# ai-forever/Kandinsky-2

Measured on NVIDIA B200. Metric: unet_denoising_steps_per_sec, higher is better.
Workload: dtype f16

## Files before the change

### kandinsky-2_b200/csrc/k2_api.cu

```cuda
#include <stdio.h>
#include <stdlib.h>
#include <string.h>

#include <algorithm>
#include <atomic>
#include <mutex>

#include "../../include/k2b200.h"
#include "k2_internal.h"

namespace k2 {

static thread_local std::string g_err;
static std::atomic<long long> g_launches{0};
static int g_force_bn = 0;
static int g_force_split = 0;
static int g_force_2cta = 0;
static int g_tail_split = 0;
static int g_attn_stagger = 1200;
static int g_attn_poly = 0;
static int g_pdl = 0;
static int g_halo_mode = 0;


// ... 99 lines not shown
        if (better) {
          best_tiles[k] = tiles;
          bn[k] = tn;
          bw[k] = tw;
          bh[k] = th;
        }
      }
    }
  }
  const int k = (!single_image_only && best_tiles[1] * 100 <= best_tiles[0] * 85) ? 1 : 0;
  TN = bn[k];
  TW = bw[k];
  TH = bh[k];
}


struct ConvPlan {
  int TN, TH, TW, tiles_w, tiles_h, tiles_n, m_tiles;
  int halo_pitch, halo_bo;
  int m_tiles_phase;
  int BN, two_cta, splits;
  int fuse_stats, row_groups;
  int es;
  int tail_first, tail_count, tail_split, tail_kps;
};

constexpr long long TAIL_FLAG_BYTES = 64 << 10;

static void plan_conv(int NB, int H, int W, bool any9, int kchunks, int Cout, int out_mode, bool has_workspace,
                      long long workspace_bytes, bool want_gn, ConvPlan& pl, const int* cfg = nullptr, bool up2 = false,
                      bool w_batched = false) {
  const int g_force_bn = (cfg && cfg[0]) ? cfg[0] : k2::g_force_bn;
  const int g_force_2cta = (cfg && cfg[1]) ? cfg[1] : k2::g_force_2cta;
  const int g_force_split = (cfg && cfg[2]) ? cfg[2] : k2::g_force_split;
  pl.es = (cfg && cfg[3]) ? cfg[3] : k2::g_conv_epi_sets;
  pl.halo_pitch = 0;
  pl.halo_bo = 0;
  if (g_halo_mode > 0 && any9 && W % 8 == 0 && H % 16 == 0 && out_mode == 0 && Cout > 64 && g_force_2cta != 1) {
    pl.halo_pitch = (g_halo_mode <= 2) ? 10 : 16;
    pl.halo_bo = (g_halo_mode == 2 || g_halo_mode == 4) ? 1 : 0;
  }
  if (pl.halo_pitch) {
    pl.TN = 1;
    pl.TH = 16;
    pl.TW = 8;
  } else {
// ... 42 lines not shown
    long long best = -1;
    int best_bn = BN ? BN : 256, best_sp = 1;
    for (int ci = 0; ci < 3; ++ci) {
      const int bn = BN ? BN : cand[ci];
      if (BN && ci > 0) break;
      for (int sp = 1; sp <= 8; ++sp) {
        if (g_force_split > 0 && sp != g_force_split) continue;
        if (pl.halo_pitch && sp > 1) continue;
        if (!split_ok(sp)) continue;
        const long long c = model(bn, sp, two_cta != 0);
        if (best < 0 || c < best) {
          best = c;
          best_bn = bn;
          best_sp = sp;
        }
      }
    }
    BN = best_bn;
    splits = best_sp;
  }
  pl.BN = BN;
  pl.two_cta = two_cta;
  pl.splits = splits;
  if (up2) {
    pl.m_tiles_phase = two_cta ? (pl.m_tiles + 1) / 2 * 2 : pl.m_tiles;
  }

  pl.tail_first = pl.tail_count = pl.tail_kps = 0;
  pl.tail_split = 1;
  if (g_tail_split && two_cta && splits == 1 && !pl.halo_pitch && out_mode == 0 && Cout % 64 == 0 && BN % 64 == 0 && has_workspace) {
    const int m_pairs = ((up2 ? 4 * pl.m_tiles_phase : pl.m_tiles) + 1) / 2;
    const int units = m_pairs * ((Cout + BN - 1) / BN);
    const int P = num_sms() / 2;
    const int R = units % P;
    if (R > 0 && kchunks >= 16) {
      long long L = (static_cast<long long>(R) * kchunks + P - 1) / P;
      L = std::max<long long>(L, (kchunks + 2) / 3);
      int max_parts = 1;
      for (int t = 0; t < R; ++t) {
        const long long first = static_cast<long long>(t) * kchunks / L;
        const long long last = std::min((static_cast<long long>(t + 1) * kchunks - 1) / L, (static_cast<long long>(R) * kchunks - 1) / L);
        max_parts = std::max(max_parts, static_cast<int>(last - first + 1));
      }
      const long long buf_bytes = static_cast<long long>(R) * 2 * 3 * 128 * BN * 4;
      const long long flag_bytes = static_cast<long long>(R) * 2 * 3 * 8 * 4;
      const long long saved_cycles = (kchunks - L) * (2LL * BN + 60);
      if ((saved_cycles >= 26000 || (g_tail_split == 2 && L < kchunks)) && max_parts <= 4 && buf_bytes <= workspace_bytes / 2 - TAIL_FLAG_BYTES &&
          flag_bytes <= TAIL_FLAG_BYTES) {
        pl.tail_first = units - R;
        pl.tail_count = R;
        pl.tail_split = 4;
        pl.tail_kps = static_cast<int>(L);
      }
    }
  }

  pl.fuse_stats = 0;
  pl.row_groups = 0;
  if (want_gn && out_mode == 0 && Cout % 8 == 0) {
    if (splits == 1 && BN >= 64 && Cout % 64 == 0 && (pl.TN == 1 || pl.TH * pl.TW == 16)) {
      pl.fuse_stats = 1;
      pl.row_groups = ((pl.TN == 1) ? pl.m_tiles : NB * pl.tiles_h * pl.tiles_w) * (up2 ? 4 : 1);
    } else if (splits > 1 && (static_cast<long long>(H) * W) % 16 == 0) {
      pl.fuse_stats = 2;
      pl.row_groups = static_cast<int>(M_total / 16);
    }
  }
}

static thread_local int g_last_tail_split = 1;
static void plan_to_info(const ConvPlan& pl, int* info) {
  g_last_tail_split = pl.tail_split;
  if (!info) return;
  info[0] = pl.BN; info[1] = pl.two_cta; info[2] = pl.splits; info[3] = pl.m_tiles; info[4] = pl.TN;
  info[5] = pl.fuse_stats; info[6] = pl.row_groups;
}

}

using namespace k2;

extern "C" {

const char* k2_last_error(void) { return g_err.c_str(); }
int k2_version(void) { return 100; }
long long k2_launch_count(void) { return g_launches.load(); }
int k2_conv_last_tail_split(void) { return g_last_tail_split; }
void k2_reset_launch_count(void) { g_launches.store(0); }
int k2_set_tuning(int key, int value) {
  if (key == 0) {
    g_force_bn = value;
    return 0;
  }
  if (key == 1) {
    g_force_split = value;
    return 0;
  }
// ... 42 lines not shown
    return 0;
  }

  return fail("k2_set_tuning: unknown key");
}

int k2_conv_gemm(const K2ConvSrc* srcs, int nsrc, int NB, int H, int W, const void* w_packed, int w_rows,
                 int Ktot, int ldw, int Cout, const float* bias, const void* residual, int ldr, void* out, int ldo,
                 int out_mode, void* workspace, long long workspace_bytes, float* gn_partial, int* info,
                 k2_stream_t stream) {
  return k2_conv_gemm_cfg(srcs, nsrc, NB, H, W, w_packed, w_rows, Ktot, ldw, Cout, bias, residual, ldr, out, ldo, out_mode,
                          workspace, workspace_bytes, gn_partial, info, nullptr, 0, stream);
}

int k2_conv_gemm_cfg(const K2ConvSrc* srcs, int nsrc, int NB, int H, int W, const void* w_packed, int w_rows,
                     int Ktot, int ldw, int Cout, const float* bias, const void* residual, int ldr, void* out, int ldo,
                     int out_mode, void* workspace, long long workspace_bytes, float* gn_partial, int* info,
                     const int* cfg, long long w_batch_stride, k2_stream_t stream) {
  K2_REQUIRE(w_batch_stride >= 0 && w_batch_stride % 8 == 0, "conv_gemm_cfg: w_batch_stride must be a multiple of 8 elements");
  const bool w_batched = w_batch_stride > 0;
  if (cfg) {
    K2_REQUIRE(cfg[0] == 0 || cfg[0] == 16 || cfg[0] == 64 || cfg[0] == 128 || cfg[0] == 192 || cfg[0] == 256,
               "conv_gemm_cfg: N tile must be 0, 16, 64, 128, 192 or 256");
    K2_REQUIRE(cfg[1] >= 0 && cfg[1] <= 2 && cfg[2] >= 0 && cfg[2] <= 8 && cfg[3] >= 0 && cfg[3] <= 2,
               "conv_gemm_cfg: pair mode in 0..2, splits in 0..8, epilogue sets in 0..2");
  }
  K2_REQUIRE(nsrc >= 1 && nsrc <= 3, "conv_gemm: 1..3 sources");
  K2_REQUIRE(NB > 0 && H > 0 && W > 0 && Cout > 0, "conv_gemm: bad geometry");
  K2_REQUIRE(w_rows >= Cout, "conv_gemm: w_rows < Cout");
  K2_REQUIRE(Ktot % 64 == 0, "conv_gemm: Ktot must be a multiple of 64");
  if (ldw == 0) ldw = Ktot;
  K2_REQUIRE(ldw >= Ktot && ldw % 8 == 0 && (reinterpret_cast<uintptr_t>(w_packed) & 15) == 0,
             "conv_gemm: weight row stride / alignment");
  ConvGemmParams p;
  memset(&p, 0, sizeof p);
  p.NB = NB;
  p.H = H;
  p.W = W;
  bool any9 = false;
  int kchunks = 0;
  const bool up2 = srcs[0].taps == 4;
  if (up2) {
    K2_REQUIRE(nsrc == 1 && out_mode == 0 && residual == nullptr && H % 2 == 0 && W % 2 == 0,
               "conv_gemm: a taps == 4 source (3x3 conv over its nearest-2x upsampling) must be the only source, with fp16 "
               "output, no residual and even output H, W");
    H /= 2;
    W /= 2;
    p.H = H;
// ... 61 lines not shown
  }
  p.n_tiles = (Cout + BN - 1) / BN;
  p.Cout = Cout;
  {
    uint64_t dims[3] = {static_cast<uint64_t>(Ktot), static_cast<uint64_t>(w_rows), static_cast<uint64_t>(w_batched ? NB : 1)};
    uint64_t str[2] = {static_cast<uint64_t>(ldw) * 2,
                       (w_batched ? static_cast<uint64_t>(w_batch_stride) : static_cast<uint64_t>(ldw) * w_rows) * 2};
    uint32_t box[3] = {64, static_cast<uint32_t>(two_cta ? BN / 2 : BN), 1};
    if (encode_tmap_f16(&p.tmB, w_packed, 3, dims, str, box)) return -1;
  }
  p.bias = bias;
  p.residual = reinterpret_cast<const __half*>(residual);
  p.ldr = ldr;
  p.out = out;
  p.ldo = ldo;
  p.out_mode = (splits > 1) ? 2 : out_mode;
  p.gn_part = (fuse_stats == 1) ? reinterpret_cast<float2*>(gn_partial) : nullptr;
  p.gn_mode = (fuse_stats == 1) ? (p.TN == 1 ? 1 : 2) : 0;
  if (out_mode == 0) {
    K2_REQUIRE(ldo % 8 == 0 && (reinterpret_cast<uintptr_t>(out) & 15) == 0, "conv_gemm: out alignment");
    if (residual)
      K2_REQUIRE(ldr % 8 == 0 && (reinterpret_cast<uintptr_t>(residual) & 15) == 0, "conv_gemm: residual alignment");
  }
  int rc = launch_conv_gemm(p, BN, pl.es, static_cast<cudaStream_t>(stream));
  if (rc == 0) g_launches.fetch_add(1, std::memory_order_relaxed);
  if (rc == 0 && splits > 1) {
    rc = launch_splitk_finalize(p.ws, splits, p.M_total, Cout, bias, p.residual, ldr, reinterpret_cast<__half*>(out), ldo,
                                fuse_stats == 2 ? reinterpret_cast<float2*>(gn_partial) : nullptr,
                                static_cast<cudaStream_t>(stream));
    if (rc == 0) g_launches.fetch_add(1, std::memory_order_relaxed);
  }
  return rc;
}

int k2_conv_plan(int NB, int H, int W, int taps, int Ktot, int Cout, int out_mode, long long workspace_bytes,
                 int want_gn_partial, int* info) {
  K2_REQUIRE(NB > 0 && H > 0 && W > 0 && Cout > 0 && info, "conv_plan: bad arguments");
  K2_REQUIRE(Ktot > 0 && Ktot % 64 == 0, "conv_plan: Ktot must be a positive multiple of 64");
  ConvPlan pl;
  plan_conv(NB, H, W, taps == 9, Ktot / 64, Cout, out_mode, workspace_bytes > 0, workspace_bytes, want_gn_partial != 0, pl);
  plan_to_info(pl, info);
  return 0;
}

}
```

### kandinsky-2_b200/csrc/k2_common.cuh

```cuda
#pragma once
#include <cuda.h>
#include <cuda_fp16.h>
#include <cuda_runtime.h>
#include <stdint.h>
#include <stdio.h>

namespace k2 {

__device__ __forceinline__ uint32_t smem_u32(const void* p) {
  return static_cast<uint32_t>(__cvta_generic_to_shared(p));
}

__device__ __forceinline__ uint32_t lane_id() { return threadIdx.x & 31; }

__device__ __forceinline__ bool elect_one() {
  uint32_t pred = 0;
  asm volatile(
      "{\n"
      ".reg .b32 rx;\n"
      ".reg .pred px;\n"
      "elect.sync rx|px, 0xffffffff;\n"
      "selp.b32 %0, 1, 0, px;\n"
      "}\n"
      : "=r"(pred));
// ... 237 lines not shown
      "cp.async.bulk.tensor.2d.cta_group::2.shared::cluster.global.mbarrier::complete_tx::bytes [%0], [%1, {%3, "
      "%4}], [%2];"
      ::"r"(smem_u32(dst)),
      "l"(reinterpret_cast<uint64_t>(tm)), "r"(smem_u32(bar) & kPeerBitMask), "r"(c0), "r"(c1)
      : "memory");
}
__device__ __forceinline__ void tma2_load_3d(void* dst, const CUtensorMap* tm, uint64_t* bar, int c0, int c1, int c2) {
  asm volatile(
      "cp.async.bulk.tensor.3d.cta_group::2.shared::cluster.global.mbarrier::complete_tx::bytes [%0], [%1, {%3, "
      "%4, %5}], [%2];"
      ::"r"(smem_u32(dst)),
      "l"(reinterpret_cast<uint64_t>(tm)), "r"(smem_u32(bar) & kPeerBitMask), "r"(c0), "r"(c1), "r"(c2)
      : "memory");
}
__device__ __forceinline__ void tma2_load_4d(void* dst, const CUtensorMap* tm, uint64_t* bar, int c0, int c1,
                                             int c2, int c3) {
  asm volatile(
      "cp.async.bulk.tensor.4d.cta_group::2.shared::cluster.global.mbarrier::complete_tx::bytes [%0], [%1, {%3, "
      "%4, %5, %6}], [%2];"
      ::"r"(smem_u32(dst)),
      "l"(reinterpret_cast<uint64_t>(tm)), "r"(smem_u32(bar) & kPeerBitMask), "r"(c0), "r"(c1), "r"(c2), "r"(c3)
      : "memory");
}
__device__ __forceinline__ void tmem_alloc2(uint32_t* smem_dst, uint32_t ncols) {
  asm volatile("tcgen05.alloc.cta_group::2.sync.aligned.shared::cta.b32 [%0], %1;" ::"r"(smem_u32(smem_dst)),
               "r"(ncols)
               : "memory");
}
__device__ __forceinline__ void tmem_relinquish2() {
  asm volatile("tcgen05.relinquish_alloc_permit.cta_group::2.sync.aligned;" ::: "memory");
}
__device__ __forceinline__ void tmem_dealloc2(uint32_t taddr, uint32_t ncols) {
  asm volatile("tcgen05.dealloc.cta_group::2.sync.aligned.b32 %0, %1;" ::"r"(taddr), "r"(ncols) : "memory");
}
__device__ __forceinline__ void umma2_f16(uint32_t tmem_d, uint64_t adesc, uint64_t bdesc, uint32_t idesc,
                                          uint32_t accumulate) {
  asm volatile(
      "{\n"
      ".reg .pred p;\n"
      "setp.ne.b32 p, %4, 0;\n"
      "tcgen05.mma.cta_group::2.kind::f16 [%0], %1, %2, %3, p;\n"
      "}\n" ::"r"(tmem_d),
      "l"(adesc), "l"(bdesc), "r"(idesc), "r"(accumulate)
      : "memory");
}
__device__ __forceinline__ void umma2_commit_mc(uint64_t* bar, uint16_t mask) {
// ... 117 lines not shown
```

### kandinsky-2_b200/csrc/k2_conv_gemm.cu

```cuda
#include <stdio.h>

#include "k2_common.cuh"
#include "k2_internal.h"

namespace k2 {

namespace {

constexpr int BM = 128;
constexpr int BK = 64;
constexpr int A_STAGE_BYTES = BM * BK * 2;

constexpr int EPI_STAGE_FLOATS = 32 * 33;
constexpr int EPI_BYTES = 4 * EPI_STAGE_FLOATS * 4 + 4 * 256 * 4;

template <int BN>
struct Cfg {
  static constexpr int B_STAGE_BYTES = BN * BK * 2;
  static constexpr int STAGE_BYTES = A_STAGE_BYTES + B_STAGE_BYTES;
  static constexpr int STAGES = (BN >= 256) ? 4 : (BN >= 192 ? 5 : (BN >= 128 ? 6 : 8));
  static constexpr int TMEM_COLS = (2 * BN <= 32) ? 32 : (2 * BN <= 64 ? 64 : (2 * BN <= 128 ? 128 : (2 * BN <= 256 ? 256 : 512)));
  static constexpr int BAR_BYTES = 256;
  static constexpr int STAT_BYTES = EPI_BYTES;
  static constexpr int SMEM_BYTES = STAGES * STAGE_BYTES + BAR_BYTES + STAT_BYTES + 1024;
// ... 511 lines not shown
      acc ^= 1;
      if (acc == 0) acc_phase ^= 1;
    }
  }

  tc_fence_before();
  __syncthreads();
  if (warp_idx == 2) {
    tc_fence_after();
    tmem_dealloc(tmem_base, C::TMEM_COLS);
  }
}

template <int BN, int ES = 1>
struct Cfg2 {
  static constexpr int B_STAGE_BYTES = (BN / 2) * BK * 2;
  static constexpr int STAGE_BYTES = A_STAGE_BYTES + B_STAGE_BYTES;
  static constexpr int STAGES = ((BN >= 256) ? 6 : (BN >= 192 ? 7 : 8)) - (ES - 1);
  static constexpr int TMEM_COLS = 512;
  static constexpr int SMEM_BYTES = STAGES * STAGE_BYTES + 256 + ES * EPI_BYTES + 1024;
  static constexpr int THREADS = 128 + 128 * ES;
};

template <int BN, int ES = 1, bool TAIL = false>
__global__ void __cluster_dims__(2, 1, 1) __launch_bounds__(128 + 128 * ES, 1)
conv_gemm2_kernel(const __grid_constant__ ConvGemmParams p) {
  using C = Cfg2<BN, ES>;
  extern __shared__ uint8_t smem_raw[];
  uint8_t* smem = reinterpret_cast<uint8_t*>((reinterpret_cast<uintptr_t>(smem_raw) + 1023) &
                                             ~static_cast<uintptr_t>(1023));
  uint64_t* full_bar = reinterpret_cast<uint64_t*>(smem + C::STAGES * C::STAGE_BYTES);
  uint64_t* empty_bar = full_bar + C::STAGES;
  uint64_t* tmem_full = empty_bar + C::STAGES;
  uint64_t* tmem_empty = tmem_full + 2;
  uint32_t* tmem_ptr = reinterpret_cast<uint32_t*>(tmem_empty + 2);
  float* stat_smem = reinterpret_cast<float*>(smem + C::STAGES * C::STAGE_BYTES + 256);

  const int warp_idx = threadIdx.x >> 5;
  const int lane = threadIdx.x & 31;
  const uint32_t rank = cluster_ctarank();
  const int pair = blockIdx.x >> 1;
  const int num_pairs = gridDim.x >> 1;

  if (warp_idx == 0 && lane == 0) {
    tma_prefetch_desc(&p.tmB);
    for (int s = 0; s < 3; ++s)
      if (p.seg_taps[s]) tma_prefetch_desc(&p.tmA[s]);
  }
  if (warp_idx == 1 && lane == 0) {
    for (int i = 0; i < C::STAGES; ++i) {
      mbar_init(&full_bar[i], 1);
      mbar_init(&empty_bar[i], 1);
    }
    for (int i = 0; i < 2; ++i) {
      mbar_init(&tmem_full[i], 1);
      mbar_init(&tmem_empty[i], 8 * ES);
    }
    fence_barrier_init();
  }
  if (warp_idx == 2) {
    tmem_alloc2(tmem_ptr, C::TMEM_COLS);
    tmem_relinquish2();
  }
  tc_fence_before();
  cluster_sync_all();
  tc_fence_after();
  const uint32_t tmem_base = *tmem_ptr;
  pdl_wait();
  pdl_launch();

  const int m_pairs = (p.m_tiles + 1) >> 1;
  const int total_tiles = TAIL ? p.tail_first + 2 * num_pairs : m_pairs * p.n_tiles * p.splits;
  auto decode_item = [&](int item, int& tile, int& part, int& nparts, int& split, int& k0, int& k1) -> bool {
    if (TAIL && item >= p.tail_first) {
      const int idx = item - p.tail_first;
      const int sub = idx / num_pairs, i = idx - sub * num_pairs;
      const int nk = p.num_k_chunks, L = p.tail_kps;
      const int g0 = i * L, g1 = min(g0 + L, p.tail_count * nk);
      if (g0 >= g1) return false;
      int ta = g0 / nk;
      const int ka0 = g0 - ta * nk, ka1 = min(nk, ka0 + (g1 - g0));
      if (sub == 0) {
        k0 = ka0;
        k1 = ka1;
      } else {
        const int rest = (g1 - g0) - (ka1 - ka0);
        if (rest <= 0) return false;
        ++ta;
        k0 = 0;
        k1 = rest;
      }
      const int first_span = (ta * nk) / L;
      const int last_span = min(((ta + 1) * nk - 1) / L, (p.tail_count * nk - 1) / L);
      part = i - first_span;
      nparts = last_span - first_span + 1;
      tile = p.tail_first + ta;
      split = 0;
      return true;
    }
    tile = item;
    part = -1;
    nparts = 1;
    split = tile / (m_pairs * p.n_tiles);
    k0 = split * p.k_per_split;
    k1 = min(p.num_k_chunks, k0 + p.k_per_split);
    return true;
  };

  if (warp_idx == 0) {
    if (elect_one()) {
      int stage = 0;
      uint32_t ring_phase = 0;
      const uint32_t tx_bytes = 2u * (p.a_box_bytes + C::B_STAGE_BYTES);
      for (int item = pair; item < total_tiles; item += num_pairs) {
        int tile, part, nparts, split, k0, k1;
        if (!decode_item(item, tile, part, nparts, split, k0, k1)) continue;
        const int m_idx = (tile % m_pairs) * 2 + static_cast<int>(rank);
        const int n_idx = (tile / m_pairs) % p.n_tiles;
        int n0, y0, x0, phase;
        decode_m_tile(p, m_idx, n0, y0, x0, phase);
        const int kb = phase * p.num_k_chunks;
        int s = 0, rem = k0;
        while (rem >= p.seg_taps[s] * p.seg_kchunks[s]) {
          rem -= p.seg_taps[s] * p.seg_kchunks[s];
          ++s;
        }
        int tap = rem / p.seg_kchunks[s];
        int c = rem - tap * p.seg_kchunks[s];
        for (int kc = k0; kc < k1; ++kc) {
          const int taps = p.seg_taps[s];
          const int dy = (taps == 9) ? (tap / 3 - 1) : (taps == 4 ? (tap >> 1) + (phase >> 1) - 1 : 0);
          const int dx = (taps == 9) ? (tap % 3 - 1) : (taps == 4 ? (tap & 1) + (phase & 1) - 1 : 0);
          mbar_wait(&empty_bar[stage], ring_phase ^ 1);
          uint8_t* sA = smem + stage * C::STAGE_BYTES;
          uint8_t* sB = sA + A_STAGE_BYTES;
          if (rank == 0) mbar_arrive_expect_tx(&full_bar[stage], tx_bytes);
          tma2_load_4d(sA, &p.tmA[s], &full_bar[stage], c * BK, x0 + dx, y0 + dy, n0);
          tma2_load_3d(sB, &p.tmB, &full_bar[stage], (kb + kc) * BK, n_idx * BN + static_cast<int>(rank) * (BN / 2),
                       p.w_batched ? n0 : 0);
          if (++stage == C::STAGES) {
            stage = 0;
            ring_phase ^= 1;
          }
          if (++c == p.seg_kchunks[s]) {
            c = 0;
            if (++tap == taps) {
              tap = 0;
              ++s;
            }
          }
        }
      }
    }
  } else if (warp_idx == 1) {
    if (rank == 0 && elect_one()) {
      constexpr uint32_t idesc = make_idesc_f16(256, BN, 0, 0);
      int stage = 0;
      uint32_t phase = 0;
      int acc = 0;
      uint32_t acc_phase = 0;
      for (int item = pair; item < total_tiles; item += num_pairs) {
        int tile, part, nparts, split, k0, k1;
        if (!decode_item(item, tile, part, nparts, split, k0, k1)) continue;
        mbar_wait(&tmem_empty[acc], acc_phase ^ 1);
        tc_fence_after();
        const uint32_t d_tmem = tmem_base + static_cast<uint32_t>(acc * 256);
        const int nk = k1 - k0;
        for (int kc = 0; kc < nk; ++kc) {
          mbar_wait(&full_bar[stage], phase);
          tc_fence_after();
          const uint32_t a_addr = smem_u32(smem + stage * C::STAGE_BYTES);
          const uint64_t adesc = make_sw128_desc(a_addr);
          const uint64_t bdesc = make_sw128_desc(a_addr + A_STAGE_BYTES);
#pragma unroll
          for (int k = 0; k < BK / 16; ++k)
            umma2_f16(d_tmem, adesc + static_cast<uint64_t>(k * 2), bdesc + static_cast<uint64_t>(k * 2), idesc,
                      (kc | k) != 0 ? 1u : 0u);
          umma2_commit_mc(&empty_bar[stage], 0x3);
          if (++stage == C::STAGES) {
            stage = 0;
            phase ^= 1;
          }
        }
        umma2_commit_mc(&tmem_full[acc], 0x3);
        acc ^= 1;
        if (acc == 0) acc_phase ^= 1;
      }
    }
  } else if (warp_idx >= 4) {
    const int ew = (ES == 1) ? warp_idx - 4 : (warp_idx & 3);
    const int es = (ES == 1) ? 0 : ((warp_idx - 4) >> 2);
    int acc = 0;
    uint32_t acc_phase = 0;
    const uint32_t leader_empty0 = mapa_u32(smem_u32(&tmem_empty[0]), 0);
    const uint32_t leader_empty1 = mapa_u32(smem_u32(&tmem_empty[1]), 0);
    for (int item = pair; item < total_tiles; item += num_pairs) {
      int tile, part, nparts, split, k0, k1;
      if (!decode_item(item, tile, part, nparts, split, k0, k1)) continue;
      const int m_idx = (tile % m_pairs) * 2 + static_cast<int>(rank);
      const int n_idx = (tile / m_pairs) % p.n_tiles;
      int n0, y0, x0, phase;
      decode_m_tile(p, m_idx, n0, y0, x0, phase);
      const int tail_role = (part < 0 || nparts == 1) ? 0 : (part > 0 ? 1 : 2);
      const int tail_slot = (part < 0) ? 0 : ((tile - p.tail_first) * 2 + static_cast<int>(rank)) * (p.tail_split - 1) + max(part - 1, 0);
      mbar_wait(&tmem_full[acc], acc_phase);
      tc_fence_after();
      epilogue_tile<BN, ES, TAIL>(p, tmem_base, acc * 256, ew, lane, n0, y0, x0, n_idx, split, m_idx, stat_smem, es, phase,
                                  tail_role, tail_slot, nparts - 1);
      tc_fence_before();
      __syncwarp();
      if (lane == 0) mbar_arrive_cluster(acc ? leader_empty1 : leader_empty0);
      acc ^= 1;
      if (acc == 0) acc_phase ^= 1;
    }
  }

  tc_fence_before();
  cluster_sync_all();
  if (warp_idx == 2) {
    tc_fence_after();
    tmem_dealloc2(tmem_base, C::TMEM_COLS);
  }
}

template <int BN, int ES, bool TAIL>
int launch_pair(const ConvGemmParams& p, cudaStream_t stream) {
  using C = Cfg2<BN, ES>;
  static bool attr_set = false;
  if (!attr_set) {
    K2_CHECK_CUDA(cudaFuncSetAttribute(conv_gemm2_kernel<BN, ES, TAIL>, cudaFuncAttributeMaxDynamicSharedMemorySize, C::SMEM_BYTES));
    attr_set = true;
  }
  const int m_pairs = (p.m_tiles + 1) / 2;
  const int total = m_pairs * p.n_tiles * p.splits;
  const int max_pairs = num_sms() / 2;
  const int pairs = (TAIL || total >= max_pairs) ? max_pairs : total;
  K2_CHECK_CUDA(launch_k(conv_gemm2_kernel<BN, ES, TAIL>, dim3(2 * pairs), dim3(C::THREADS), C::SMEM_BYTES, stream, p));
  return 0;
}
template <int BN>
int launch_bn2(const ConvGemmParams& p, cudaStream_t stream) {
  return p.tail_split > 1 ? launch_pair<BN, 1, true>(p, stream) : launch_pair<BN, 1, false>(p, stream);
}
template <int BN>
int launch_bn2e(const ConvGemmParams& p, cudaStream_t stream) {
  return p.tail_split > 1 ? launch_pair<BN, 2, true>(p, stream) : launch_pair<BN, 2, false>(p, stream);
}

template <int BN>
struct Cfg3 {
  static constexpr int A_STAGE = 36864;
  static constexpr int A_STAGES = 3;
  static constexpr int B_STAGE = (BN / 2) * BK * 2;
  static constexpr int B_STAGES = (BN >= 256) ? 4 : 5;
  static constexpr int BAR_OFF = A_STAGES * A_STAGE + B_STAGES * B_STAGE;
  static constexpr int STAT_OFF = BAR_OFF + 256;
  static constexpr int SMEM_BYTES = STAT_OFF + EPI_BYTES + 1024;
};

template <int BN>
__global__ void __cluster_dims__(2, 1, 1) __launch_bounds__(256, 1)
conv_gemm3_kernel(const __grid_constant__ ConvGemmParams p) {
  using C = Cfg3<BN>;
  extern __shared__ uint8_t smem_raw[];
  uint8_t* smem = reinterpret_cast<uint8_t*>((reinterpret_cast<uintptr_t>(smem_raw) + 1023) &
                                             ~static_cast<uintptr_t>(1023));
  uint8_t* smemB = smem + C::A_STAGES * C::A_STAGE;
  uint64_t* a_full = reinterpret_cast<uint64_t*>(smem + C::BAR_OFF);
  uint64_t* a_empty = a_full + C::A_STAGES;
// ... 265 lines not shown
  using C = Cfg<BN>;
  static bool attr_set = false;
  if (!attr_set) {
    K2_CHECK_CUDA(cudaFuncSetAttribute(conv_gemm_kernel<BN>, cudaFuncAttributeMaxDynamicSharedMemorySize,
                                       C::SMEM_BYTES));
    attr_set = true;
  }
  int total = p.m_tiles * p.n_tiles * p.splits;
  int grid = total < num_sms() ? total : num_sms();
  K2_CHECK_CUDA(launch_k(conv_gemm_kernel<BN>, dim3(grid), dim3(256), C::SMEM_BYTES, stream, p));
  return 0;
}

}

int launch_splitk_finalize(const float* ws, int splits, long long M, int Cout, const float* bias, const __half* residual,
                           int ldr, __half* out, int ldo, float2* gn_part, cudaStream_t stream) {
  dim3 grid(static_cast<unsigned int>((M + 15) / 16), (Cout / 8 + 31) / 32);
  K2_CHECK_CUDA(launch_k(splitk_finalize_kernel, grid, dim3(256), 0, stream, ws, splits, M, Cout, bias, residual, ldr, out, ldo,
                         gn_part));
  return 0;
}

int launch_conv_gemm(const ConvGemmParams& p, int BN, int epilogue_sets, cudaStream_t stream) {
  if (p.halo_pitch) {
    switch (BN) {
      case 128: return launch_bn3<128>(p, stream);
      case 192: return launch_bn3<192>(p, stream);
      case 256: return launch_bn3<256>(p, stream);
      default: return fail("conv_gemm: unsupported BN for the halo kernel");
    }
  }
  if (p.two_cta && epilogue_sets == 2) {
    switch (BN) {
      case 128: return launch_bn2e<128>(p, stream);
      case 192: return launch_bn2e<192>(p, stream);
      case 256: return launch_bn2e<256>(p, stream);
      default: return fail("conv_gemm: unsupported BN for the 2-CTA kernel");
    }
  }
  if (p.two_cta) {
    switch (BN) {
      case 128: return launch_bn2<128>(p, stream);
      case 192: return launch_bn2<192>(p, stream);
      case 256: return launch_bn2<256>(p, stream);
      default: return fail("conv_gemm: unsupported BN for the 2-CTA kernel");
    }
  }
  switch (BN) {
    case 16: return launch_bn<16>(p, stream);
    case 64: return launch_bn<64>(p, stream);
    case 128: return launch_bn<128>(p, stream);
    case 192: return launch_bn<192>(p, stream);
    case 256: return launch_bn<256>(p, stream);
    default: return fail("conv_gemm: unsupported BN");
  }
}

}
```

### kandinsky-2_b200/csrc/k2_internal.h

```cpp
#pragma once
#include <cuda.h>
#include <cuda_fp16.h>
#include <cuda_runtime.h>
#include <stdint.h>

#include <string>

namespace k2 {

void set_error(const std::string& msg);
int fail(const std::string& msg);
#define K2_CHECK_CUDA(expr)                                                                 \
  do {                                                                                      \
    cudaError_t _e = (expr);                                                                \
    if (_e != cudaSuccess)                                                                  \
      return ::k2::fail(std::string(#expr) + ": " + cudaGetErrorString(_e));                \
  } while (0)
#define K2_REQUIRE(cond, msg)                                  \
  do {                                                         \
    if (!(cond)) return ::k2::fail(std::string("k2b200: ") + (msg)); \
  } while (0)

int num_sms();
bool pdl_enabled();
// ... 32 lines not shown
  int Cout;
  const float* bias;
  const __half* residual;
  int ldr;
  void* out;
  int ldo;
  int out_mode;
  uint32_t a_box_bytes;
  int splits;
  int k_per_split;
  float* ws;
  long long M_total;
  int two_cta;
  float2* gn_part;
  int gn_mode;
  int up2;
  int m_tiles_phase;
  int halo_pitch;
  int halo_bo;
  int tail_first, tail_count, tail_split, tail_kps;
  float* tail_buf;
  unsigned int* tail_flags;
};
int launch_conv_gemm(const ConvGemmParams& p, int BN, int epilogue_sets, cudaStream_t stream);
int launch_splitk_finalize(const float* ws, int splits, long long M, int Cout, const float* bias, const __half* residual,
                           int ldr, __half* out, int ldo, float2* gn_part, cudaStream_t stream);

struct AttnParams {
  CUtensorMap tmQKV;
  CUtensorMap tmEnc;
  int B, heads, T, Tc;
  int hs, q_off, k_off, v_off;
  int ehs, ek_off, ev_off;
  __half* out;
  int ldo;
  float scale_log2e;
  int stagger_cycles;
  unsigned long long* trace;
};
int gn_apply_blocks_per_sm();
int attention_stagger();
unsigned long long* attention_trace_buffer();
int attention_half_rows();
int attention_poly_mode();
int launch_attention_d64(const AttnParams& p, cudaStream_t stream);

}
// ... 1 lines not shown
```

### kandinsky-2_b200/kandinsky2/launch_plan.py

```python
import os

import torch

from . import ops

FOLD_MAX_RG = int(os.environ.get("K2_GN_FOLD_MAX_RG", "18"))
TUNE = os.environ.get("K2_AUTOTUNE", "1") != "0"
FORK = os.environ.get("K2_FORK", "1") != "0"
TUNE_SMALL_M = int(os.environ.get("K2_TUNE_SMALL_M", "8192"))
_tune_cache = {}


def tune(key, run, m_rows=0):
    if not TUNE:
        return None
    key = (torch.cuda.current_device(), TUNE_SMALL_M) + key
    if key in _tune_cache:
        return _tune_cache[key]
    info = [0] * 7
    run(None, info)
    bn0, pair, splits = info[0], info[1], info[2]
    best = None
    if pair:
        cout = key[3]
        bns = [bn0] if splits > 1 else [bn for bn in (128, 192, 256) if bn - 64 < cout or bn == bn0]
        cands = [(bn0, 0, splits, 1)] + [(bn, 0, splits, es) for bn in bns for es in (1, 2) if (bn, es) != (bn0, 1)]
        if 0 < m_rows <= TUNE_SMALL_M and splits == 1:
            for pm in (2, 1):
                for bn in (128, 192, 256):
                    if bn - 64 >= cout:
                        continue
                    for sp in ((2, 3, 4) if pm == 2 else (1, 2, 3, 4)):
                        probe = [0] * 7
                        try:
                            run((bn, pm, sp, 1), probe)
                        except Exception:
                            continue
                        if probe[0] == bn and probe[2] == sp and bool(probe[1]) == (pm == 2):
                            cands.append((bn, pm, sp, 1))

        def timed(cfg, reps=6):
            run(cfg)
            evs = [torch.cuda.Event(enable_timing=True) for _ in range(reps + 1)]
            evs[0].record()
            for i in range(reps):
                run(cfg)
                evs[i + 1].record()
            torch.cuda.synchronize()
            return min(evs[i].elapsed_time(evs[i + 1]) for i in range(reps))
# ... 172 lines not shown
```

### profiles/ab_step.py

```python
import argparse
import os
import statistics
import sys

ROOT = os.path.dirname(os.path.dirname(os.path.abspath(__file__)))
sys.path.insert(0, ROOT)
sys.path.insert(0, os.path.join(ROOT, "kandinsky-2_b200"))
import torch

import bench
from kandinsky2 import launch_plan, ops
from kandinsky2.model import unet as unet_mod
from kandinsky2.model.gaussian_diffusion import FusedStep, create_ddpm_v22


TUNING_DEFAULTS = {4: 1, 5: 1200, 9: 1, 12: 0}


def main():
    ap = argparse.ArgumentParser()
    ap.add_argument("variants", nargs="+")
    ap.add_argument("--rounds", type=int, default=5)
    ap.add_argument("--steps", type=int, default=20)
    ap.add_argument("--hw", default="96x96")
    ap.add_argument("--batch", type=int, default=4)
    ap.add_argument("--profile", action="store_true", help="also print the per-kind eager event sums of each variant")
    args = ap.parse_args()
    H, W = (int(v) for v in args.hw.split("x"))
    B = args.batch
    dev = torch.device("cuda", 0)
    ops.set_tuning(4, 1)
    model = unet_mod.Text2ImUNet(**bench.UNET_CFG, device=dev, param_dtype=torch.float16)
    model.init_synthetic_(seed=0)
    model.finalize(release_params=True)
    emb = torch.randn(2 * B, 1280, device=dev)
    diffusion = create_ddpm_v22(50)
    coef, ts = diffusion._tables(dev)
    steps = []
    for spec in args.variants:
        kv = dict(item.split("=") for item in spec.split(",") if item)
        launch_plan.FOLD_MAX_RG = int(kv.get("fold", launch_plan.FOLD_MAX_RG))
        launch_plan.TUNE = kv.get("tune", "1") != "0"
        launch_plan.FORK = kv.get("fork", "1") != "0"
        launch_plan.TUNE_SMALL_M = int(kv.get("smallm", "8192"))
        if hasattr(unet_mod, "_UP2"):
            unet_mod._UP2 = kv.get("up2", "1") != "0"
        tkeys = {int(k[1:]): int(v) for k, v in kv.items() if k[0] == "t" and k[1:].isdigit()}
        for k, v in tkeys.items():
            ops.set_tuning(k, v)
        model._plans = {}
        if kv.get("repack"):
            model.finalize()
        st = FusedStep(model, B, H, W, dict(image_emb=emb), guidance_scale=4.0, cond_first=False, clip_range=2.0,
                       threshold_mode=0)
        x = torch.randn(B, 4, H, W, device=dev)
        if kv.get("drop"):
            dropped = set(kv["drop"].split("+"))
            st.plan.steps = [s for s in st.plan.steps if s[1] not in dropped]
            st.plan.graph = None
        for n in range(3):
            st.noise.normal_()
            st.run(x, ts[40], coef[40])
        for k in tkeys:
            ops.set_tuning(k, TUNING_DEFAULTS.get(k, 0))
        steps.append((spec, st, x))
    torch.cuda.synchronize()
    times = {spec: [] for spec, _, _ in steps}
# ... 23 lines not shown
```

Before: 62.22.

## Add 4-CTA cluster A-operand TMA multicast variant to the conv GEMM autotuner

Adds an optional conv GEMM mode in which two CTA pairs that work on adjacent N tiles form a 4-CTA cluster. Each pair loads alternate K chunks of the shared A (activation) tile and multicasts them to both pairs, which halves A traffic from L2. Pairs whose N tile is out of range still take part in the barriers but skip MMA and epilogue work. The mode is added to the autotuner candidate list by default. The cost is the extra cross-pair synchronisation, with empty barriers counting two arrivals, and a smaller number of resident cluster units.

```diff
diff --git a/kandinsky-2_b200/csrc/k2_api.cu b/kandinsky-2_b200/csrc/k2_api.cu
--- a/kandinsky-2_b200/csrc/k2_api.cu
+++ b/kandinsky-2_b200/csrc/k2_api.cu
@@ -145,6 +145,7 @@
   int BN, two_cta, splits;
   int fuse_stats, row_groups;
   int es;
+  int mc;
   int tail_first, tail_count, tail_split, tail_kps;
 };
 
@@ -233,13 +234,14 @@
   pl.BN = BN;
   pl.two_cta = two_cta;
   pl.splits = splits;
+  pl.mc = (g_force_2cta == 3 && two_cta && !pl.halo_pitch && (Cout + BN - 1) / BN >= 2) ? 1 : 0;
   if (up2) {
     pl.m_tiles_phase = two_cta ? (pl.m_tiles + 1) / 2 * 2 : pl.m_tiles;
   }
 
   pl.tail_first = pl.tail_count = pl.tail_kps = 0;
   pl.tail_split = 1;
-  if (g_tail_split && two_cta && splits == 1 && !pl.halo_pitch && out_mode == 0 && Cout % 64 == 0 && BN % 64 == 0 && has_workspace) {
+  if (g_tail_split && two_cta && !pl.mc && splits == 1 && !pl.halo_pitch && out_mode == 0 && Cout % 64 == 0 && BN % 64 == 0 && has_workspace) {
     const int m_pairs = ((up2 ? 4 * pl.m_tiles_phase : pl.m_tiles) + 1) / 2;
     const int units = m_pairs * ((Cout + BN - 1) / BN);
     const int P = num_sms() / 2;
@@ -283,7 +285,7 @@
 static void plan_to_info(const ConvPlan& pl, int* info) {
   g_last_tail_split = pl.tail_split;
   if (!info) return;
-  info[0] = pl.BN; info[1] = pl.two_cta; info[2] = pl.splits; info[3] = pl.m_tiles; info[4] = pl.TN;
+  info[0] = pl.BN; info[1] = pl.two_cta ? 1 + pl.mc : 0; info[2] = pl.splits; info[3] = pl.m_tiles; info[4] = pl.TN;
   info[5] = pl.fuse_stats; info[6] = pl.row_groups;
 }
 
@@ -372,8 +374,8 @@
   if (cfg) {
     K2_REQUIRE(cfg[0] == 0 || cfg[0] == 16 || cfg[0] == 64 || cfg[0] == 128 || cfg[0] == 192 || cfg[0] == 256,
                "conv_gemm_cfg: N tile must be 0, 16, 64, 128, 192 or 256");
-    K2_REQUIRE(cfg[1] >= 0 && cfg[1] <= 2 && cfg[2] >= 0 && cfg[2] <= 8 && cfg[3] >= 0 && cfg[3] <= 2,
-               "conv_gemm_cfg: pair mode in 0..2, splits in 0..8, epilogue sets in 0..2");
+    K2_REQUIRE(cfg[1] >= 0 && cfg[1] <= 3 && cfg[2] >= 0 && cfg[2] <= 8 && cfg[3] >= 0 && cfg[3] <= 2,
+               "conv_gemm_cfg: pair mode in 0..3, splits in 0..8, epilogue sets in 0..2");
   }
   K2_REQUIRE(nsrc >= 1 && nsrc <= 3, "conv_gemm: 1..3 sources");
   K2_REQUIRE(NB > 0 && H > 0 && W > 0 && Cout > 0, "conv_gemm: bad geometry");
@@ -481,7 +483,7 @@
     if (residual)
       K2_REQUIRE(ldr % 8 == 0 && (reinterpret_cast<uintptr_t>(residual) & 15) == 0, "conv_gemm: residual alignment");
   }
-  int rc = launch_conv_gemm(p, BN, pl.es, static_cast<cudaStream_t>(stream));
+  int rc = launch_conv_gemm(p, BN, pl.es, pl.mc != 0, static_cast<cudaStream_t>(stream));
   if (rc == 0) g_launches.fetch_add(1, std::memory_order_relaxed);
   if (rc == 0 && splits > 1) {
     rc = launch_splitk_finalize(p.ws, splits, p.M_total, Cout, bias, p.residual, ldr, reinterpret_cast<__half*>(out), ldo,
diff --git a/kandinsky-2_b200/csrc/k2_common.cuh b/kandinsky-2_b200/csrc/k2_common.cuh
--- a/kandinsky-2_b200/csrc/k2_common.cuh
+++ b/kandinsky-2_b200/csrc/k2_common.cuh
@@ -283,6 +283,15 @@
       "l"(reinterpret_cast<uint64_t>(tm)), "r"(smem_u32(bar) & kPeerBitMask), "r"(c0), "r"(c1), "r"(c2), "r"(c3)
       : "memory");
 }
+__device__ __forceinline__ void tma2_load_4d_mc(void* dst, const CUtensorMap* tm, uint64_t* bar, uint16_t mask, int c0,
+                                                int c1, int c2, int c3) {
+  asm volatile(
+      "cp.async.bulk.tensor.4d.cta_group::2.shared::cluster.global.mbarrier::complete_tx::bytes.multicast::cluster [%0], "
+      "[%1, {%4, %5, %6, %7}], [%2], %3;"
+      ::"r"(smem_u32(dst)),
+      "l"(reinterpret_cast<uint64_t>(tm)), "r"(smem_u32(bar) & kPeerBitMask), "h"(mask), "r"(c0), "r"(c1), "r"(c2), "r"(c3)
+      : "memory");
+}
 __device__ __forceinline__ void tmem_alloc2(uint32_t* smem_dst, uint32_t ncols) {
   asm volatile("tcgen05.alloc.cta_group::2.sync.aligned.shared::cta.b32 [%0], %1;" ::"r"(smem_u32(smem_dst)),
                "r"(ncols)
diff --git a/kandinsky-2_b200/csrc/k2_conv_gemm.cu b/kandinsky-2_b200/csrc/k2_conv_gemm.cu
--- a/kandinsky-2_b200/csrc/k2_conv_gemm.cu
+++ b/kandinsky-2_b200/csrc/k2_conv_gemm.cu
@@ -557,9 +557,10 @@
   static constexpr int THREADS = 128 + 128 * ES;
 };
 
-template <int BN, int ES = 1, bool TAIL = false>
-__global__ void __cluster_dims__(2, 1, 1) __launch_bounds__(128 + 128 * ES, 1)
+template <int BN, int ES = 1, bool TAIL = false, bool MC = false>
+__global__ void __cluster_dims__(MC ? 4 : 2, 1, 1) __launch_bounds__(128 + 128 * ES, 1)
 conv_gemm2_kernel(const __grid_constant__ ConvGemmParams p) {
+  static_assert(!(MC && TAIL), "A multicast and the tail split are exclusive");
   using C = Cfg2<BN, ES>;
   extern __shared__ uint8_t smem_raw[];
   uint8_t* smem = reinterpret_cast<uint8_t*>((reinterpret_cast<uintptr_t>(smem_raw) + 1023) &
@@ -573,9 +574,11 @@
 
   const int warp_idx = threadIdx.x >> 5;
   const int lane = threadIdx.x & 31;
-  const uint32_t rank = cluster_ctarank();
-  const int pair = blockIdx.x >> 1;
-  const int num_pairs = gridDim.x >> 1;
+  const uint32_t crank = cluster_ctarank();
+  const uint32_t rank = MC ? (crank & 1u) : crank;
+  const uint32_t mc_pair = MC ? (crank >> 1) : 0u;
+  const int pair = MC ? blockIdx.x >> 2 : blockIdx.x >> 1;
+  const int num_pairs = MC ? gridDim.x >> 2 : gridDim.x >> 1;
 
   if (warp_idx == 0 && lane == 0) {
     tma_prefetch_desc(&p.tmB);
@@ -585,7 +588,7 @@
   if (warp_idx == 1 && lane == 0) {
     for (int i = 0; i < C::STAGES; ++i) {
       mbar_init(&full_bar[i], 1);
-      mbar_init(&empty_bar[i], 1);
+      mbar_init(&empty_bar[i], MC ? 2 : 1);
     }
     for (int i = 0; i < 2; ++i) {
       mbar_init(&tmem_full[i], 1);
@@ -605,7 +608,9 @@
   pdl_launch();
 
   const int m_pairs = (p.m_tiles + 1) >> 1;
-  const int total_tiles = TAIL ? p.tail_first + 2 * num_pairs : m_pairs * p.n_tiles * p.splits;
+  const int n_groups = MC ? (p.n_tiles + 1) >> 1 : p.n_tiles;
+  const int total_tiles = TAIL ? p.tail_first + 2 * num_pairs : m_pairs * n_groups * p.splits;
+  auto n_tile_of = [&](int tile) { return ((tile / m_pairs) % n_groups) * (MC ? 2 : 1) + static_cast<int>(mc_pair); };
   auto decode_item = [&](int item, int& tile, int& part, int& nparts, int& split, int& k0, int& k1) -> bool {
     if (TAIL && item >= p.tail_first) {
       const int idx = item - p.tail_first;
@@ -636,7 +641,7 @@
     tile = item;
     part = -1;
     nparts = 1;
-    split = tile / (m_pairs * p.n_tiles);
+    split = tile / (m_pairs * n_groups);
     k0 = split * p.k_per_split;
     k1 = min(p.num_k_chunks, k0 + p.k_per_split);
     return true;
@@ -651,7 +656,8 @@
         int tile, part, nparts, split, k0, k1;
         if (!decode_item(item, tile, part, nparts, split, k0, k1)) continue;
         const int m_idx = (tile % m_pairs) * 2 + static_cast<int>(rank);
-        const int n_idx = (tile / m_pairs) % p.n_tiles;
+        const int n_idx = n_tile_of(tile);
+        const bool live = !MC || n_idx < p.n_tiles;
         int n0, y0, x0, phase;
         decode_m_tile(p, m_idx, n0, y0, x0, phase);
         const int kb = phase * p.num_k_chunks;
@@ -669,10 +675,19 @@
           mbar_wait(&empty_bar[stage], ring_phase ^ 1);
           uint8_t* sA = smem + stage * C::STAGE_BYTES;
           uint8_t* sB = sA + A_STAGE_BYTES;
-          if (rank == 0) mbar_arrive_expect_tx(&full_bar[stage], tx_bytes);
-          tma2_load_4d(sA, &p.tmA[s], &full_bar[stage], c * BK, x0 + dx, y0 + dy, n0);
-          tma2_load_3d(sB, &p.tmB, &full_bar[stage], (kb + kc) * BK, n_idx * BN + static_cast<int>(rank) * (BN / 2),
-                       p.w_batched ? n0 : 0);
+          if constexpr (MC) {
+            if (rank == 0) mbar_arrive_expect_tx(&full_bar[stage], live ? tx_bytes : 2u * p.a_box_bytes);
+            if ((kc & 1) == static_cast<int>(mc_pair))
+              tma2_load_4d_mc(sA, &p.tmA[s], &full_bar[stage], static_cast<uint16_t>(0x5u << rank), c * BK, x0 + dx, y0 + dy, n0);
+            if (live)
+              tma2_load_3d(sB, &p.tmB, &full_bar[stage], (kb + kc) * BK, n_idx * BN + static_cast<int>(rank) * (BN / 2),
+                           p.w_batched ? n0 : 0);
+          } else {
+            if (rank == 0) mbar_arrive_expect_tx(&full_bar[stage], tx_bytes);
+            tma2_load_4d(sA, &p.tmA[s], &full_bar[stage], c * BK, x0 + dx, y0 + dy, n0);
+            tma2_load_3d(sB, &p.tmB, &full_bar[stage], (kb + kc) * BK, n_idx * BN + static_cast<int>(rank) * (BN / 2),
+                         p.w_batched ? n0 : 0);
+          }
           if (++stage == C::STAGES) {
             stage = 0;
             ring_phase ^= 1;
@@ -686,10 +701,21 @@
           }
         }
       }
+      if constexpr (MC) {
+        for (int i = 0; i < C::STAGES; ++i) {
+          mbar_wait(&empty_bar[stage], ring_phase ^ 1);
+          if (++stage == C::STAGES) {
+            stage = 0;
+            ring_phase ^= 1;
+          }
+        }
+      }
     }
   } else if (warp_idx == 1) {
     if (rank == 0 && elect_one()) {
       constexpr uint32_t idesc = make_idesc_f16(256, BN, 0, 0);
+      constexpr uint16_t kStageMask = MC ? 0xF : 0x3;
+      const uint16_t acc_mask = static_cast<uint16_t>(0x3u << (2 * mc_pair));
       int stage = 0;
       uint32_t phase = 0;
       int acc = 0;
@@ -697,6 +723,7 @@
       for (int item = pair; item < total_tiles; item += num_pairs) {
         int tile, part, nparts, split, k0, k1;
         if (!decode_item(item, tile, part, nparts, split, k0, k1)) continue;
+        const bool live = !MC || n_tile_of(tile) < p.n_tiles;
         mbar_wait(&tmem_empty[acc], acc_phase ^ 1);
         tc_fence_after();
         const uint32_t d_tmem = tmem_base + static_cast<uint32_t>(acc * 256);
@@ -707,17 +734,19 @@
           const uint32_t a_addr = smem_u32(smem + stage * C::STAGE_BYTES);
           const uint64_t adesc = make_sw128_desc(a_addr);
           const uint64_t bdesc = make_sw128_desc(a_addr + A_STAGE_BYTES);
-#pragma unroll
-          for (int k = 0; k < BK / 16; ++k)
-            umma2_f16(d_tmem, adesc + static_cast<uint64_t>(k * 2), bdesc + static_cast<uint64_t>(k * 2), idesc,
-                      (kc | k) != 0 ? 1u : 0u);
-          umma2_commit_mc(&empty_bar[stage], 0x3);
+          if (live) {
+#pragma unroll
+            for (int k = 0; k < BK / 16; ++k)
+              umma2_f16(d_tmem, adesc + static_cast<uint64_t>(k * 2), bdesc + static_cast<uint64_t>(k * 2), idesc,
+                        (kc | k) != 0 ? 1u : 0u);
+          }
+          umma2_commit_mc(&empty_bar[stage], kStageMask);
           if (++stage == C::STAGES) {
             stage = 0;
             phase ^= 1;
           }
         }
-        umma2_commit_mc(&tmem_full[acc], 0x3);
+        umma2_commit_mc(&tmem_full[acc], acc_mask);
         acc ^= 1;
         if (acc == 0) acc_phase ^= 1;
       }
@@ -727,21 +756,22 @@
     const int es = (ES == 1) ? 0 : ((warp_idx - 4) >> 2);
     int acc = 0;
     uint32_t acc_phase = 0;
-    const uint32_t leader_empty0 = mapa_u32(smem_u32(&tmem_empty[0]), 0);
-    const uint32_t leader_empty1 = mapa_u32(smem_u32(&tmem_empty[1]), 0);
+    const uint32_t leader_empty0 = mapa_u32(smem_u32(&tmem_empty[0]), 2 * mc_pair);
+    const uint32_t leader_empty1 = mapa_u32(smem_u32(&tmem_empty[1]), 2 * mc_pair);
     for (int item = pair; item < total_tiles; item += num_pairs) {
       int tile, part, nparts, split, k0, k1;
       if (!decode_item(item, tile, part, nparts, split, k0, k1)) continue;
       const int m_idx = (tile % m_pairs) * 2 + static_cast<int>(rank);
-      const int n_idx = (tile / m_pairs) % p.n_tiles;
+      const int n_idx = n_tile_of(tile);
       int n0, y0, x0, phase;
       decode_m_tile(p, m_idx, n0, y0, x0, phase);
       const int tail_role = (part < 0 || nparts == 1) ? 0 : (part > 0 ? 1 : 2);
       const int tail_slot = (part < 0) ? 0 : ((tile - p.tail_first) * 2 + static_cast<int>(rank)) * (p.tail_split - 1) + max(part - 1, 0);
       mbar_wait(&tmem_full[acc], acc_phase);
       tc_fence_after();
-      epilogue_tile<BN, ES, TAIL>(p, tmem_base, acc * 256, ew, lane, n0, y0, x0, n_idx, split, m_idx, stat_smem, es, phase,
-                                  tail_role, tail_slot, nparts - 1);
+      if (!MC || n_idx < p.n_tiles)
+        epilogue_tile<BN, ES, TAIL>(p, tmem_base, acc * 256, ew, lane, n0, y0, x0, n_idx, split, m_idx, stat_smem, es, phase,
+                                    tail_role, tail_slot, nparts - 1);
       tc_fence_before();
       __syncwarp();
       if (lane == 0) mbar_arrive_cluster(acc ? leader_empty1 : leader_empty0);
@@ -758,28 +788,36 @@
   }
 }
 
-template <int BN, int ES, bool TAIL>
+template <int BN, int ES, bool TAIL, bool MC = false>
 int launch_pair(const ConvGemmParams& p, cudaStream_t stream) {
   using C = Cfg2<BN, ES>;
-  static bool attr_set = false;
-  if (!attr_set) {
-    K2_CHECK_CUDA(cudaFuncSetAttribute(conv_gemm2_kernel<BN, ES, TAIL>, cudaFuncAttributeMaxDynamicSharedMemorySize, C::SMEM_BYTES));
-    attr_set = true;
+  auto* kernel = conv_gemm2_kernel<BN, ES, TAIL, MC>;
+  static int max_units = 0;
+  if (!max_units) {
+    K2_CHECK_CUDA(cudaFuncSetAttribute(kernel, cudaFuncAttributeMaxDynamicSharedMemorySize, C::SMEM_BYTES));
+    if (MC) {
+      cudaLaunchConfig_t cfg = {};
+      cfg.gridDim = dim3(4 * (num_sms() / 4));
+      cfg.blockDim = dim3(C::THREADS);
+      cfg.dynamicSmemBytes = C::SMEM_BYTES;
+      int clusters = 0;
+      K2_CHECK_CUDA(cudaOccupancyMaxActiveClusters(&clusters, kernel, &cfg));
+      K2_REQUIRE(clusters > 0, "conv_gemm: no 4-CTA cluster of the A-multicast kernel fits on this device");
+      max_units = clusters;
+    } else {
+      max_units = num_sms() / 2;
+    }
   }
   const int m_pairs = (p.m_tiles + 1) / 2;
-  const int total = m_pairs * p.n_tiles * p.splits;
-  const int max_pairs = num_sms() / 2;
-  const int pairs = (TAIL || total >= max_pairs) ? max_pairs : total;
-  K2_CHECK_CUDA(launch_k(conv_gemm2_kernel<BN, ES, TAIL>, dim3(2 * pairs), dim3(C::THREADS), C::SMEM_BYTES, stream, p));
+  const int total = m_pairs * (MC ? (p.n_tiles + 1) / 2 : p.n_tiles) * p.splits;
+  const int units = (TAIL || total >= max_units) ? max_units : total;
+  K2_CHECK_CUDA(launch_k(kernel, dim3((MC ? 4 : 2) * units), dim3(C::THREADS), C::SMEM_BYTES, stream, p));
   return 0;
 }
-template <int BN>
-int launch_bn2(const ConvGemmParams& p, cudaStream_t stream) {
-  return p.tail_split > 1 ? launch_pair<BN, 1, true>(p, stream) : launch_pair<BN, 1, false>(p, stream);
-}
-template <int BN>
-int launch_bn2e(const ConvGemmParams& p, cudaStream_t stream) {
-  return p.tail_split > 1 ? launch_pair<BN, 2, true>(p, stream) : launch_pair<BN, 2, false>(p, stream);
+template <int BN, int ES>
+int launch_bn2(const ConvGemmParams& p, bool mc, cudaStream_t stream) {
+  if (mc) return launch_pair<BN, ES, false, true>(p, stream);
+  return p.tail_split > 1 ? launch_pair<BN, ES, true>(p, stream) : launch_pair<BN, ES, false>(p, stream);
 }
 
 template <int BN>
@@ -1091,7 +1129,7 @@
   return 0;
 }
 
-int launch_conv_gemm(const ConvGemmParams& p, int BN, int epilogue_sets, cudaStream_t stream) {
+int launch_conv_gemm(const ConvGemmParams& p, int BN, int epilogue_sets, bool a_multicast, cudaStream_t stream) {
   if (p.halo_pitch) {
     switch (BN) {
       case 128: return launch_bn3<128>(p, stream);
@@ -1102,20 +1140,21 @@
   }
   if (p.two_cta && epilogue_sets == 2) {
     switch (BN) {
-      case 128: return launch_bn2e<128>(p, stream);
-      case 192: return launch_bn2e<192>(p, stream);
-      case 256: return launch_bn2e<256>(p, stream);
+      case 128: return launch_bn2<128, 2>(p, a_multicast, stream);
+      case 192: return launch_bn2<192, 2>(p, a_multicast, stream);
+      case 256: return launch_bn2<256, 2>(p, a_multicast, stream);
       default: return fail("conv_gemm: unsupported BN for the 2-CTA kernel");
     }
   }
   if (p.two_cta) {
     switch (BN) {
-      case 128: return launch_bn2<128>(p, stream);
-      case 192: return launch_bn2<192>(p, stream);
-      case 256: return launch_bn2<256>(p, stream);
+      case 128: return launch_bn2<128, 1>(p, a_multicast, stream);
+      case 192: return launch_bn2<192, 1>(p, a_multicast, stream);
+      case 256: return launch_bn2<256, 1>(p, a_multicast, stream);
       default: return fail("conv_gemm: unsupported BN for the 2-CTA kernel");
     }
   }
+  if (a_multicast) return fail("conv_gemm: A multicast needs the CTA-pair kernel");
   switch (BN) {
     case 16: return launch_bn<16>(p, stream);
     case 64: return launch_bn<64>(p, stream);
diff --git a/kandinsky-2_b200/csrc/k2_internal.h b/kandinsky-2_b200/csrc/k2_internal.h
--- a/kandinsky-2_b200/csrc/k2_internal.h
+++ b/kandinsky-2_b200/csrc/k2_internal.h
@@ -78,7 +78,7 @@
   float* tail_buf;
   unsigned int* tail_flags;
 };
-int launch_conv_gemm(const ConvGemmParams& p, int BN, int epilogue_sets, cudaStream_t stream);
+int launch_conv_gemm(const ConvGemmParams& p, int BN, int epilogue_sets, bool a_multicast, cudaStream_t stream);
 int launch_splitk_finalize(const float* ws, int splits, long long M, int Cout, const float* bias, const __half* residual,
                            int ldr, __half* out, int ldo, float2* gn_part, cudaStream_t stream);
 
diff --git a/kandinsky-2_b200/kandinsky2/launch_plan.py b/kandinsky-2_b200/kandinsky2/launch_plan.py
--- a/kandinsky-2_b200/kandinsky2/launch_plan.py
+++ b/kandinsky-2_b200/kandinsky2/launch_plan.py
@@ -8,13 +8,15 @@
 TUNE = os.environ.get("K2_AUTOTUNE", "1") != "0"
 FORK = os.environ.get("K2_FORK", "1") != "0"
 TUNE_SMALL_M = int(os.environ.get("K2_TUNE_SMALL_M", "8192"))
+TUNE_MC = os.environ.get("K2_TUNE_MC", "1") != "0"
 _tune_cache = {}
 
 
 def tune(key, run, m_rows=0):
     if not TUNE:
         return None
-    key = (torch.cuda.current_device(), TUNE_SMALL_M) + key
+    cout = key[1]
+    key = (torch.cuda.current_device(), TUNE_SMALL_M, TUNE_MC) + key
     if key in _tune_cache:
         return _tune_cache[key]
     info = [0] * 7
@@ -22,9 +24,10 @@
     bn0, pair, splits = info[0], info[1], info[2]
     best = None
     if pair:
-        cout = key[3]
         bns = [bn0] if splits > 1 else [bn for bn in (128, 192, 256) if bn - 64 < cout or bn == bn0]
         cands = [(bn0, 0, splits, 1)] + [(bn, 0, splits, es) for bn in bns for es in (1, 2) if (bn, es) != (bn0, 1)]
+        if TUNE_MC:
+            cands += [(bn, 3, splits, es) for bn in bns for es in (1, 2) if bn < cout]
         if 0 < m_rows <= TUNE_SMALL_M and splits == 1:
             for pm in (2, 1):
                 for bn in (128, 192, 256):
diff --git a/profiles/ab_step.py b/profiles/ab_step.py
--- a/profiles/ab_step.py
+++ b/profiles/ab_step.py
@@ -43,6 +43,7 @@
         launch_plan.TUNE = kv.get("tune", "1") != "0"
         launch_plan.FORK = kv.get("fork", "1") != "0"
         launch_plan.TUNE_SMALL_M = int(kv.get("smallm", "8192"))
+        launch_plan.TUNE_MC = kv.get("mc", "1") != "0"
         if hasattr(unet_mod, "_UP2"):
             unet_mod._UP2 = kv.get("up2", "1") != "0"
         tkeys = {int(k[1:]): int(v) for k, v in kv.items() if k[0] == "t" and k[1:].isdigit()}
diff --git a/profiles/mc_probe.py b/profiles/mc_probe.py
--- /dev/null
+++ b/profiles/mc_probe.py
@@ -0,0 +1,109 @@
+import os
+import statistics
+import sys
+
+ROOT = os.path.dirname(os.path.dirname(os.path.abspath(__file__)))
+sys.path.insert(0, ROOT)
+sys.path.insert(0, os.path.join(ROOT, "kandinsky-2_b200"))
+import torch
+
+from kandinsky2 import ops
+
+SHAPES = [
+    ("L0 conv3x3 384->384 96x96", 8, 96, 96, [(384, 9)], 384, False, 14),
+    ("L1 conv3x3 768->768 48x48", 8, 48, 48, [(768, 9)], 768, True, 16),
+    ("L1 qkv 18432x768 -> 2304", 1, 1, 18432, [(768, 1)], 2304, False, 7),
+    ("L1 proj 18432x768 -> 768 +res", 1, 1, 18432, [(768, 1)], 768, True, 7),
+    ("L2 conv3x3 1152->1152 24x24", 8, 24, 24, [(1152, 9)], 1152, True, 16),
+    ("L2 up conv3x3 1152 + skip 1152|768", 8, 24, 24, [(1152, 9), (1152, 1), (768, 1)], 1152, False, 3),
+    ("L2 qkv 4608x1152 -> 3456", 1, 1, 4608, [(1152, 1)], 3456, False, 7),
+    ("L3 conv3x3 1536->1536 12x12", 8, 12, 12, [(1536, 9)], 1536, True, 18),
+    ("L3 qkv 1152x1536 -> 4608", 1, 1, 1152, [(1536, 1)], 4608, False, 8),
+]
+
+
+def timed(fn, reps=30):
+    for _ in range(3):
+        fn()
+    evs = [torch.cuda.Event(enable_timing=True) for _ in range(reps + 1)]
+    evs[0].record()
+    for i in range(reps):
+        fn()
+        evs[i + 1].record()
+    torch.cuda.synchronize()
+    return statistics.median(evs[i].elapsed_time(evs[i + 1]) for i in range(reps)) * 1e3
+
+
+def l2_bytes(info, nk, cout, mc):
+    bn, m_tiles = info[0], info[3]
+    units = (m_tiles + 1) // 2 * -(-cout // bn)
+    a = 2 * 16384 // (2 if mc else 1)
+    return units * nk * (a + bn * 128)
+
+
+def plan_choices():
+    import bench
+    from kandinsky2 import launch_plan
+    from kandinsky2.model import unet as unet_mod
+    from kandinsky2.model.gaussian_diffusion import FusedStep, create_ddpm_v22
+    dev = torch.device("cuda", 0)
+    ops.set_tuning(4, 1)
+    model = unet_mod.Text2ImUNet(**bench.UNET_CFG, device=dev, param_dtype=torch.float16)
+    model.init_synthetic_(seed=0)
+    model.finalize(release_params=True)
+    B = 4
+    coef, ts = create_ddpm_v22(50)._tables(dev)
+    st = FusedStep(model, B, 96, 96, dict(image_emb=torch.randn(2 * B, 1280, device=dev)), guidance_scale=4.0, cond_first=False,
+                   clip_range=2.0, threshold_mode=0)
+    x = torch.randn(B, 4, 96, 96, device=dev)
+    st.run(x, ts[40], coef[40])
+    torch.cuda.synchronize()
+    for key, cfg in launch_plan._tune_cache.items():
+        print(f"{'MC ' if cfg and cfg[1] == 3 else '   '} {cfg}  {key[3:]}")
+
+
+def main():
+    if "--plan" in sys.argv:
+        return plan_choices()
+    energy = "--energy" in sys.argv
+    if energy:
+        sys.path.insert(0, os.path.join(ROOT, "profiles"))
+        import energy_probe
+    g = torch.Generator(device="cuda").manual_seed(0)
+    print(f"{torch.cuda.get_device_name(0)}")
+    for name, NB, H, W, srcs_spec, cout, res, cnt in SHAPES:
+        srcs = [(torch.randn(NB, H, W, c, device="cuda", generator=g).half(), taps) for c, taps in srcs_spec]
+        ktot = sum(-(-c // 64) * 64 * taps for c, taps in srcs_spec)
+        nk = ktot // 64
+        wp = (torch.randn(cout, ktot, device="cuda", generator=g) / ktot ** 0.5).half()
+        bias = torch.randn(cout, device="cuda", generator=g)
+        r = torch.randn(NB, H, W, cout, device="cuda", generator=g).half() if res else None
+        y = torch.empty(NB, H, W, cout, device="cuda", dtype=torch.float16)
+        info = [0] * 7
+        ops.conv_gemm(srcs, wp, cout, bias=bias, residual=r, out=y, info=info)
+        torch.cuda.synchronize()
+        flops = 2 * NB * H * W * ktot * cout
+        print(f"== {name}: library choice N tile {info[0]}, pair {info[1]}, splits {info[2]}, {info[3]} M tiles", flush=True)
+        for bn in (128, 192, 256):
+            if bn - 64 >= cout:
+                continue
+            line = f"   BN {bn:3d}"
+            for mode in (2, 3):
+                cfg = (bn, mode, info[2], 1)
+                probe = [0] * 7
+                ops.conv_gemm(srcs, wp, cout, bias=bias, residual=r, out=y, info=probe, cfg=cfg)
+                if mode == 3 and probe[1] != 2:
+                    line += "  mc: n/a (one N tile)"
+                    continue
+                fn = lambda: ops.conv_gemm(srcs, wp, cout, bias=bias, residual=r, out=y, cfg=cfg)
+                us = timed(fn)
+                mb = l2_bytes(probe, -(-nk // probe[2]) * probe[2], cout, mode == 3) / 1e6
+                line += f"  {'mc  ' if mode == 3 else 'pair'} {us:8.1f} us {flops / us / 1e6:5.0f} TFLOP/s L2->SM {mb:7.1f} MB"
+                if energy:
+                    _, pw, mhz = energy_probe.measure(f"      {name} BN {bn} {'mc' if mode == 3 else 'pair'}", fn, cnt, seconds=1.0)
+                    line += f" {pw * us * 1e-3:7.2f} mJ @ {mhz} MHz"
+            print(line, flush=True)
+
+
+if __name__ == "__main__":
+    main()
```

After: 62.91 (median of 6 runs). No clear change (+1.1%).
